# michaelnny/muzero

Measured on AMD Instinct MI355X. Metric: self-play MCTS sims/sec (env-steps/sec = value / sims_per_move), higher is better.
Workload: dtype f32

## Files before the change

### muzero_amd/csrc/mz_env.h

```cpp
#pragma once
#include "mz_device.h"

namespace mz {

constexpr int ENV_CARTPOLE = 1;
constexpr int ENV_TICTACTOE = 2;
constexpr int ENV_GOMOKU = 3;
constexpr int ENV_SYNTHETIC = 4;

struct EnvState {
    int kind, B, A, D, ring_len;
    int bn, nn, win;
    double* cp_state;
    int* steps;
    unsigned int* episode;
    double* init_state;
    signed char* board;
    signed char* planes;
    int* player;
    float* r_obs;
    int* r_action;
    float* r_reward;
    double* r_pi;
    double* r_root;
// ... 471 lines not shown
        if (cell) {
            mine[i] = nm0; mine[nn + i] = m0; mine[2 * nn + i] = m1; mine[3 * nn + i] = m2;
            o[0 * nn + i] = (float)t0; o[1 * nn + i] = (float)nm0;
            o[2 * nn + i] = (float)t1; o[3 * nn + i] = (float)m0;
            o[4 * nn + i] = (float)t2; o[5 * nn + i] = (float)m1;
            o[6 * nn + i] = (float)t3; o[7 * nn + i] = (float)m2;
            o[8 * nn + i] = opp == 1 ? 1.0f : 0.0f;
            if (i == a) { b[i] = (signed char)me; L.mask[(size_t)e * (nn + 1) + a] = 0; }
        }
        if (lane == 0) {
            L.env.player[e] = opp;
            L.env.steps[e] = st + 1;
            L.cur[e] = opp;
            L.opp[e] = me;
        }
    } else {
        if (cell) {
            b[i] = 0;
#pragma unroll
            for (int t = 0; t < 8; t++) { pl[t * nn + i] = 0; o[t * nn + i] = 0.0f; }
            o[8 * nn + i] = 1.0f;
            L.mask[(size_t)e * (nn + 1) + i] = 1;
        }
        if (lane == 0) {
            L.mask[(size_t)e * (nn + 1) + nn] = 1;
            atomicAdd(&L.env.counters[2], 1ULL);
            atomicAdd(&L.env.counters[3], (unsigned long long)(st + 1));
            L.env.steps[e] = 0;
            L.env.episode[e] += 1;
            L.env.player[e] = 1;
            L.cur[e] = 1;
            L.opp[e] = 2;
        }
    }
    const size_t rec = (size_t)L.slot * L.B + e;
    if (lane < A) L.env.r_pi[rec * A + lane] = pi[lane];
    if (lane == 0) {
        L.env.r_action[rec] = a;
        L.env.r_reward[rec] = reward;
        L.env.r_root[rec] = root;
        L.env.r_done[rec] = done ? 1 : 0;
        if (e == 0) {
            atomicAdd(&L.env.counters[0], (unsigned long long)L.B);
            atomicAdd(&L.env.counters[1], (unsigned long long)L.B * (unsigned long long)L.sims);
        }
    }
}

__device__ inline void env_step_group(const EnvLaunch& L, int e, int lane) {
    if (L.env.kind != ENV_TICTACTOE && L.env.kind != ENV_GOMOKU) {
        if (lane == 0) env_step_one(L, e);
        return;
    }
    const int a = __shfl(lane == 0 ? L.action[e] : 0, 0, 16);
    float reward;
    bool done;
    if (L.env.nn <= 16) board_step_small(L, e, lane, a, reward, done);
    else board_step_group(L, e, lane, a, reward, done);
    if (lane == 0) env_record(L, e, a, reward, done);
}

__global__ void k_env_step(const EnvLaunch L) {
    const int g = blockIdx.x * blockDim.x + threadIdx.x;
    if ((g >> 4) < L.B) env_step_group(L, g >> 4, g & 15);
}

struct ReplayRing {
    long long capacity;
    float* state;
    signed char* action;
    int action16;
    float* pi_prob;
    float* value;
    float* reward;
    float* priority;
    long long* num_added;
    long long* ctr;
    int* off;
    int* origin;
    int acc, K, td, board;
    double pw[34];
};

struct EpiLaunch {
    EnvState env;
    ReplayRing ring;
    int B;
    long long move_abs;
};

__device__ inline void epi_emit(const EpiLaunch& E, int e, long long start, int T, int n, long long base, long long keep_from, double* z, int lane) {
    const EnvState& V = E.env;
    const ReplayRing& R = E.ring;
    const int B = E.B, A = V.A, D = V.D, K = R.K;
    auto rec = [&](int i) { return (size_t)((start + i) % V.ring_len) * B + e; };
    if (R.board) {
        const double fr = (double)V.r_reward[rec(T - 1)];
        const int fp = V.r_player[rec(T - 1)];
        for (int t = lane; t < T; t += 64) z[t] = fr != 0.0 ? (V.r_player[rec(t)] == fp ? fr : -fr) : 0.0;
    } else {
        for (int t = lane; t < T; t += 64) {
            double acc = 0.0;
            for (int i = 0; i < R.td; i++) acc = acc + R.pw[i] * (t + i < T ? (double)V.r_reward[rec(t + i)] : 0.0);
            z[t] = acc + R.pw[R.td] * (t + R.td < T ? V.r_root[rec(t + R.td)] : 0.0);
        }
    }
    __syncthreads();
    for (int j = lane; j < n * D; j += 64) {
        const int t = j / D, i = j - t * D;
        if (base + t < keep_from) continue;
        R.state[(size_t)((base + t) % R.capacity) * D + i] = V.r_obs[rec(t) * D + i];
    }
    for (int j = lane; j < n * K; j += 64) {
        const int t = j / K, k = j - t * K, idx = t + k;
        if (base + t < keep_from) continue;
        const size_t o = (size_t)((base + t) % R.capacity) * K + k;
        const bool real = idx < T;
        if (R.action16) reinterpret_cast<short*>(R.action)[o] = real ? (short)V.r_action[rec(idx)] : (short)0;
        else R.action[o] = real ? (signed char)V.r_action[rec(idx)] : (signed char)0;
        R.reward[o] = real ? V.r_reward[rec(idx)] : 0.0f;
        R.value[o] = real ? (float)z[idx] : 0.0f;
    }
    for (int j = lane; j < n * K * A; j += 64) {
        const int t = j / (K * A), r = j - t * K * A, k = r / A, a = r - k * A, idx = t + k;
        if (base + t < keep_from) continue;
        R.pi_prob[((size_t)((base + t) % R.capacity) * K + k) * A + a] = idx < T ? (float)V.r_pi[rec(idx) * A + a] : (float)(1.0 / (double)A);
    }
    for (int t = lane; t < n; t += 64) {
        if (base + t < keep_from) continue;
        const size_t slot = (size_t)((base + t) % R.capacity);
        const double d = V.r_root[rec(t)] - z[t];
        R.priority[slot] = (float)(d < 0.0 ? -d : d);
        if (R.origin) R.origin[slot] = e;
    }
    __syncthreads();
}

__global__ __launch_bounds__(64) void k_epilogue(const EpiLaunch E) {
    extern __shared__ double z[];
    const int e = blockIdx.x, lane = threadIdx.x;
    const EnvState& V = E.env;
    const ReplayRing& R = E.ring;
    long long start = V.ep_start[e];
    int len = (int)(E.move_abs + 1 - start);
    const bool done = V.r_done[(size_t)(E.move_abs % V.ring_len) * E.B + e] != 0;
    const bool flush = !R.board && len == R.acc + R.K + R.td;
    if (flush || done) {
        long long base = R.ctr[0] + (long long)R.off[e];
        const long long keep_from = R.ctr[0] + R.ctr[1] - (long long)R.capacity;
        if (flush) {
            epi_emit(E, e, start, len, R.acc, base, keep_from, z, lane);
            start += R.acc;
            len -= R.acc;
            base += R.acc;
        }
        if (done) {
            epi_emit(E, e, start, len, len, base, keep_from, z, lane);
            start = E.move_abs + 1;
        }
        if (lane == 0) V.ep_start[e] = start;
    }
}

__global__ __launch_bounds__(1024) void k_epi_scan(const EpiLaunch E) {
    __shared__ int part[1024];
    const EnvState& V = E.env;
    const ReplayRing& R = E.ring;
    const int t = threadIdx.x, per = (E.B + 1023) / 1024, e0 = t * per, e1 = e0 + per < E.B ? e0 + per : E.B;
    int sum = 0;
    for (int e = e0; e < e1; e++) {
        int len = (int)(E.move_abs + 1 - V.ep_start[e]);
        const bool done = V.r_done[(size_t)(E.move_abs % V.ring_len) * E.B + e] != 0;
        const bool flush = !R.board && len == R.acc + R.K + R.td;
        int n = 0;
        if (flush) { n += R.acc; len -= R.acc; }
        if (done) n += len;
        R.off[e] = sum;
        sum += n;
    }
    part[t] = sum;
    __syncthreads();
    for (int d = 1; d < 1024; d <<= 1) {
        const int v = t >= d ? part[t - d] : 0;
        __syncthreads();
        part[t] += v;
        __syncthreads();
    }
    const int base = part[t] - sum;
    for (int e = e0; e < e1; e++) R.off[e] += base;
    if (t == 1023) R.ctr[1] = (long long)part[1023];
}

__global__ void k_epi_publish(const ReplayRing R) {
    const long long c = R.ctr[0] + R.ctr[1];
    R.ctr[0] = c;
    *reinterpret_cast<volatile long long*>(R.num_added) = c;
}

}
```

### muzero_amd/csrc/planner.hip

```cpp
#include <hip/hip_runtime.h>

#include <cmath>
#include <cstdio>
#include <cstdlib>
#include <cstring>
#include <map>
#include <string>
#include <vector>

#include "../../include/mzplanner.h"
#include "mz_env.h"
#include "mz_arena.h"
#include "mz_extenv.h"
#include "mz_search.h"
#include "mz_search_fast.h"
#include "mz_convnet.h"

using namespace mz;

static thread_local std::string g_err;

static int fail(int code, const std::string& msg) {
    g_err = msg;
    return code;
// ... 70 lines not shown
    int n_chunks_f32 = 0, n_chunks_w3 = 0;
    PackSrc *d_srcs = nullptr, *h_srcs = nullptr;
    void **d_dst = nullptr, **h_dst = nullptr;
    hipEvent_t ev_in = nullptr, ev_out = nullptr;
    long long bytes_read = 0, bytes_written = 0;
    void free_maps() {
        for (void* b : {(void*)d_map, (void*)d_chunks_f32, (void*)d_chunks_w3, (void*)d_srcs, (void*)d_dst})
            if (b) (void)hipFree(b);
        if (h_srcs) (void)hipHostFree(h_srcs);
        if (h_dst) (void)hipHostFree(h_dst);
        d_map = nullptr; d_chunks_f32 = d_chunks_w3 = nullptr; d_srcs = h_srcs = nullptr; d_dst = h_dst = nullptr;
        n_chunks_f32 = n_chunks_w3 = 0;
        maps_valid = false;
    }
};

struct mz_planner {
    mz_config cfg;
    int device = 0;
    hipStream_t stream = nullptr;
    std::map<std::string, HostTensor> params;
    bool committed = false;

    MlpNet net{};
    MlpLds o{};
    float* d_w[L_COUNT] = {};
    float* d_b[L_COUNT] = {};
    SearchParams sp{};
    SearchParams sp2{};
    bool tree2_ok = false;
    int lds_mode0 = 0, lds_mode2 = 0;
    SearchParams sp2f{};
    bool tree2f_ok = false;
    int lds_mode2f = 0, fast_delta = 0;
    double* d_ftab_tri = nullptr;
    InferParams ip{};
    FastKey fast{};
    bool fast_mse = false;
    bool fast_layout = false;
    bool tree_old = false;
    bool force_generic = false;
    int hwx = -1;
    std::string last_dispatch = "none yet";
    float* d_stream[1] = {};
    float* d_bias_all = nullptr;
    double *d_dbg_noise = nullptr, *d_dbg_utie = nullptr, *d_dbg_ufinal = nullptr;
    FastWeights fw{};

    float* d_obs = nullptr;
    unsigned char* d_mask = nullptr;
    int *d_cur = nullptr, *d_opp = nullptr;
    double* d_temp = nullptr;
    double *d_noise = nullptr, *d_utie = nullptr, *d_ufinal = nullptr;
    float* d_hidden = nullptr;
    double* d_ftab = nullptr;
    int* d_action = nullptr;
    double *d_pi = nullptr, *d_root = nullptr;
    int* d_visits = nullptr;
    int* d_err = nullptr;
    long long* d_stamps = nullptr;
    float *d_spi0 = nullptr, *d_svalues = nullptr, *d_srewards = nullptr;
    int *d_tparent = nullptr, *d_taction = nullptr;
    float *d_inf_in = nullptr, *d_inf_hidden = nullptr, *d_inf_reward = nullptr, *d_inf_value = nullptr, *d_inf_pi = nullptr;
    int* d_inf_action = nullptr;
    int inf_cap = 0;

    bool conv = false;
    bool hbm_tree = false;
    SearchParams spg{};
    float* d_pi_scratch = nullptr;
    ConvNetDev cnet{};
    unsigned char* d_regions = nullptr;
    float *d_pi0 = nullptr, *d_sim_reward = nullptr, *d_sim_value = nullptr;
    const float** d_srcptrs = nullptr;
    float **d_dstptrs = nullptr, **d_rootptrs = nullptr;
    int* d_sim_action = nullptr;

    EnvState env{};
    int env_kind = MZ_ENV_NONE;
    unsigned int move_counter = 0;
    int ring_len = 0, ring_pos = 0, ring_count = 0;
    bool has_replay = false;
    ReplayRing replay{};
    int* d_epi_off = nullptr;
    long long* d_epi_ctr = nullptr;
    long long selfplay_moves = 0;
    ExtEnv ext{};
    int ext_od = 0;
    bool ext_pending = false;
    bool ext_broken = false;
    void* h_ext_frames = nullptr;
    unsigned char *h_ext_mask = nullptr, *h_ext_done = nullptr;
    int *h_ext_cur = nullptr, *h_ext_opp = nullptr, *h_ext_action = nullptr, *h_ext_err = nullptr;
    float* h_ext_reward = nullptr;

    ArenaState arena{};
    bool arena_open = false;
    int arena_ply = 0;
    mz_planner* arena_q = nullptr;
    hipEvent_t ev_arena_pre = nullptr, ev_arena_q = nullptr;

    struct PackState* pk = nullptr;

    bool profiling = false;
    hipEvent_t ev_begin = nullptr, ev_end = nullptr;
    std::vector<std::pair<hipEvent_t, hipEvent_t>> kev;
    size_t kev_used = 0;
};

static int obs_dim(const mz_config& c) { return c.obs_c * c.obs_h * c.obs_w; }
static int pad16(int x) { return (x + 15) & ~15; }

extern "C" const char* mz_last_error(void) { return g_err.c_str(); }
extern "C" const char* mz_version(void) { return "mzplanner 0.1 (gfx950)"; }

static thread_local std::string g_describe;
extern "C" const char* mz_planner_describe(mz_planner* p) {
    if (!p) return "null planner";
    char b[512];
    const ConvSwitches& cs = conv_switches();
    snprintf(b, sizeof b,
             "; switches: MZ_FORCE_GENERIC=%d MZ_HWX=%d MZ_TREE_OLD=%d MZ_HBM_TREE=%d"
             " | per process: MZ_ACTION_SPARSE=%d MZ_ACTION_FUSE=%d MZ_CONV_SPEC=%d MZ_TOWER=%d MZ_CONV_TILE=%d MZ_CONV_G=%d MZ_CONV_NCT=%d",
             (int)p->force_generic, p->hwx, (int)p->tree_old, (int)p->hbm_tree, cs.action_sparse, cs.action_fuse, cs.conv_spec, cs.tower, cs.conv_tile, cs.conv_g, cs.conv_nct);
    g_describe = "search: " + p->last_dispatch + b;
    if (p->conv && p->cnet.split)
        g_describe += std::string(" | conv_precision=bf16x3: ") + split_geometry(p->cnet.hh, p->cnet.hw, p->cnet.P).name + ", one launch per conv";
    else if (p->conv) g_describe += " | conv_precision=f32";
    return g_describe.c_str();
}

static void compute_layout(mz_planner* p) {
    const mz_config& c = p->cfg;
    MlpNet& n = p->net;
    n.in_dim = obs_dim(c); n.A = c.num_actions; n.P = c.num_planes; n.H = c.hidden_dim;
    n.Sv = c.value_support_size; n.Sr = c.reward_support_size;
    n.in_pad = pad16(n.in_dim); n.h_pad = pad16(n.H); n.x_pad = n.h_pad + pad16(n.A); n.p_pad = pad16(n.P);
    const int dims[L_COUNT][2] = {{n.P, n.in_dim}, {n.H, n.P}, {n.P, n.H + n.A}, {n.H, n.P}, {n.P, n.H},
                                  {n.Sr, n.P},     {n.P, n.H}, {n.A, n.P},       {n.P, n.H}, {n.Sv, n.P}};
    for (int l = 0; l < L_COUNT; l++) {
        MlpLayer& L = n.L[l];
        L.n = dims[l][0]; L.k = dims[l][1];
        L.n_tiles = (L.n + 15) / 16;
        if (l == L_DYN0) {
            const int ab = (n.A + 15) / 16, a_last = n.A - 16 * (ab - 1);
            L.kg = n.h_pad / 16 + ab;
            L.last_steps = (a_last + 3) / 4;
        } else {
            L.kg = (L.k + 15) / 16;
            const int rem = L.k - 16 * (L.kg - 1);
            L.last_steps = rem < 4 ? rem : 4;
        }
        L.split = (l == L_REP1 || l == L_DYN1 || l == L_REW1 || l == L_POL1 || l == L_VAL1) ? 1 : 0;
        L.kq = (L.kg + 3) / 4;
    }
    MlpLds& o = p->o;
    int off = 0;
    const int xk = n.in_pad > n.x_pad ? n.in_pad : n.x_pad;
    o.X = off; off += xk * 16;
    o.H1 = off; off += n.p_pad * 16;
    o.V1 = off; off += n.p_pad * 16;
    o.HN = off; off += n.h_pad * 16;
    o.HS = off; off += n.h_pad * 16;
    int mx = n.A; mx = n.Sv > mx ? n.Sv : mx; mx = n.Sr > mx ? n.Sr : mx;
    o.lg_stride = pad16(mx) + 1;
    o.LG = off; off += ((2 * 16 * o.lg_stride + 3) & ~3);
// ... 969 lines not shown
static int upload_roots(mz_planner* p, int batch, const float* h_obs, const uint8_t* h_mask, const int32_t* h_cur, const int32_t* h_opp,
                        const double* h_temp, const mz_rng_inputs* rng, int deterministic) {
    const mz_config& c = p->cfg;
    const size_t B = (size_t)batch, A = (size_t)c.num_actions;
    if (h_obs) HIPCHK(hipMemcpyAsync(p->d_obs, h_obs, B * obs_dim(c) * sizeof(float), hipMemcpyHostToDevice, p->stream));
    if (h_mask) HIPCHK(hipMemcpyAsync(p->d_mask, h_mask, B * A, hipMemcpyHostToDevice, p->stream));
    HIPCHK(hipMemcpyAsync(p->d_cur, h_cur, B * sizeof(int), hipMemcpyHostToDevice, p->stream));
    HIPCHK(hipMemcpyAsync(p->d_opp, h_opp, B * sizeof(int), hipMemcpyHostToDevice, p->stream));
    HIPCHK(hipMemcpyAsync(p->d_temp, h_temp, B * sizeof(double), hipMemcpyHostToDevice, p->stream));
    if (rng) {
        const bool want_noise = !deterministic && c.root_dirichlet_alpha > 0.0 && c.root_exploration_eps > 0.0;
        if (want_noise) {
            if (!rng->h_noise) return fail(MZ_E_INVALID, "rng inputs given but h_noise is NULL while the search mixes Dirichlet noise");
            HIPCHK(hipMemcpyAsync(p->d_noise, rng->h_noise, B * A * sizeof(double), hipMemcpyHostToDevice, p->stream));
        }
        if (!rng->h_u_tie || (!deterministic && !rng->h_u_final)) return fail(MZ_E_INVALID, "rng inputs need h_u_tie and h_u_final");
        HIPCHK(hipMemcpyAsync(p->d_utie, rng->h_u_tie, B * (size_t)c.max_ties * sizeof(double), hipMemcpyHostToDevice, p->stream));
        if (rng->h_u_final) HIPCHK(hipMemcpyAsync(p->d_ufinal, rng->h_u_final, B * sizeof(double), hipMemcpyHostToDevice, p->stream));
    }
    return MZ_OK;
}

static int download_results(mz_planner* p, int batch, int32_t* h_action, double* h_pi, double* h_root, int32_t* h_visits) {
    const size_t B = (size_t)batch, A = (size_t)p->cfg.num_actions;
    int err = 0;
    if (h_action) HIPCHK(hipMemcpyAsync(h_action, p->d_action, B * sizeof(int), hipMemcpyDeviceToHost, p->stream));
    if (h_pi) HIPCHK(hipMemcpyAsync(h_pi, p->d_pi, B * A * sizeof(double), hipMemcpyDeviceToHost, p->stream));
    if (h_root) HIPCHK(hipMemcpyAsync(h_root, p->d_root, B * sizeof(double), hipMemcpyDeviceToHost, p->stream));
    if (h_visits) HIPCHK(hipMemcpyAsync(h_visits, p->d_visits, B * A * sizeof(int), hipMemcpyDeviceToHost, p->stream));
    HIPCHK(hipMemcpyAsync(&err, p->d_err, sizeof(int), hipMemcpyDeviceToHost, p->stream));
    HIPCHK(hipStreamSynchronize(p->stream));
    if (err) {
        HIPCHK(hipMemsetAsync(p->d_err, 0, sizeof(int), p->stream));
        HIPCHK(hipStreamSynchronize(p->stream));
        if (err == 4) return fail(MZ_E_TIES, "injected tie-break stream exhausted (raise mz_config.max_ties)");
        return fail(MZ_E_INVALID, "search kernel reported error " + std::to_string(err));
    }
    return MZ_OK;
}

extern "C" int mz_planner_search(mz_planner* p, int32_t batch, const float* h_obs, const uint8_t* h_mask, const int32_t* h_cur,
                                 const int32_t* h_opp, const double* h_temp, int32_t deterministic, const mz_rng_inputs* rng,
                                 int32_t* h_action, double* h_pi, double* h_root, int32_t* h_visits) {
    if (!p || !h_obs || !h_cur || !h_opp || !h_temp || !h_action || !h_pi || !h_root) return fail(MZ_E_INVALID, "null argument to mz_planner_search");
    if (batch < 1 || batch > p->cfg.num_envs) return fail(MZ_E_INVALID, "batch exceeds mz_config.num_envs");
    if (!p->committed) return fail(MZ_E_STATE, "weights not committed");
    HIPCHK(hipSetDevice(p->device));
    int rc = upload_roots(p, batch, h_obs, h_mask, h_cur, h_opp, h_temp, rng, deterministic);
    if (rc) return rc;
    rc = launch_search(p, batch, deterministic, h_mask != nullptr, rng != nullptr, false);
    if (rc) return rc;
    return download_results(p, batch, h_action, h_pi, h_root, h_visits);
}

extern "C" int mz_planner_search_scripted(mz_planner* p, int32_t batch, const float* h_pi0, const float* h_values, const float* h_rewards,
                                          const uint8_t* h_mask, const int32_t* h_cur, const int32_t* h_opp, const double* h_temp,
                                          int32_t deterministic, const mz_rng_inputs* rng, int32_t* h_action, double* h_pi, double* h_root,
                                          int32_t* h_visits, int32_t* h_tparent, int32_t* h_taction) {
    if (!p || !h_pi0 || !h_values || !h_rewards || !h_cur || !h_opp || !h_temp || !h_action || !h_pi || !h_root)
        return fail(MZ_E_INVALID, "null argument to mz_planner_search_scripted");
    if (batch < 1 || batch > p->cfg.num_envs) return fail(MZ_E_INVALID, "batch exceeds mz_config.num_envs");
    HIPCHK(hipSetDevice(p->device));
    const size_t B = (size_t)p->cfg.num_envs, A = (size_t)p->cfg.num_actions, S = (size_t)p->cfg.num_simulations;
    if (!p->d_spi0) {
        HIPCHK(hipMalloc(&p->d_spi0, B * A * sizeof(float)));
        HIPCHK(hipMalloc(&p->d_svalues, B * S * sizeof(float)));
        HIPCHK(hipMalloc(&p->d_srewards, B * S * sizeof(float)));
        HIPCHK(hipMalloc(&p->d_tparent, B * S * sizeof(int)));
        HIPCHK(hipMalloc(&p->d_taction, B * S * sizeof(int)));
    }
    const size_t b = (size_t)batch;
    HIPCHK(hipMemcpyAsync(p->d_spi0, h_pi0, b * A * sizeof(float), hipMemcpyHostToDevice, p->stream));
    HIPCHK(hipMemcpyAsync(p->d_svalues, h_values, b * S * sizeof(float), hipMemcpyHostToDevice, p->stream));
    HIPCHK(hipMemcpyAsync(p->d_srewards, h_rewards, b * S * sizeof(float), hipMemcpyHostToDevice, p->stream));
    int rc = upload_roots(p, batch, nullptr, h_mask, h_cur, h_opp, h_temp, rng, deterministic);
    if (rc) return rc;
    rc = launch_search(p, batch, deterministic, h_mask != nullptr, rng != nullptr, true);
    if (rc) return rc;
    if (h_tparent) HIPCHK(hipMemcpyAsync(h_tparent, p->d_tparent, b * S * sizeof(int), hipMemcpyDeviceToHost, p->stream));
    if (h_taction) HIPCHK(hipMemcpyAsync(h_taction, p->d_taction, b * S * sizeof(int), hipMemcpyDeviceToHost, p->stream));
    return download_results(p, batch, h_action, h_pi, h_root, h_visits);
}

static void ring_start(mz_planner* p, int max_steps) {
    const mz_config& c = p->cfg;
    p->ring_len = (size_t)c.num_envs * obs_dim(c) * sizeof(float) * 64 > ((size_t)4 << 30) ? 16 : 64;
    if (p->has_replay) {
        const int window = p->replay.acc + p->replay.K + p->replay.td;
        int need = c.is_board_game ? c.num_actions + 1 : window;
        if (max_steps > 0) {
            const int capped = max_steps + (c.is_board_game ? 1 : p->replay.K + p->replay.td);
            need = c.is_board_game ? capped : (window < capped ? window : capped);
        }
        if (need > p->ring_len) p->ring_len = (need + 7) & ~7;
    }
    p->selfplay_moves = 0;
    p->ring_pos = 0;
    p->ring_count = 0;
}

static int ring_finish_move(mz_planner* p) {
    if (p->has_replay) {
        EpiLaunch E{};
        E.env = p->env; E.ring = p->replay; E.B = p->cfg.num_envs; E.move_abs = p->selfplay_moves;
        hipLaunchKernelGGL(k_epi_scan, dim3(1), dim3(1024), 0, p->stream, E);
        hipLaunchKernelGGL(k_epilogue, dim3(p->cfg.num_envs), dim3(64), (size_t)p->ring_len * sizeof(double), p->stream, E);
        hipLaunchKernelGGL(k_epi_publish, dim3(1), dim3(1), 0, p->stream, p->replay);
    }
    HIPCHK(hipGetLastError());
    p->selfplay_moves++;
    p->ring_pos = (p->ring_pos + 1) % p->ring_len;
    if (p->ring_count < p->ring_len) p->ring_count++;
    return MZ_OK;
}

extern "C" int mz_selfplay_reset(mz_planner* p, int32_t env_kind, const double* h_init_state) {
    if (!p) return fail(MZ_E_INVALID, "null planner");
    HIPCHK(hipSetDevice(p->device));
    const mz_config& c = p->cfg;
    int board_n = 3, num_to_win = 3;
    if (env_kind == MZ_ENV_CARTPOLE) {
        if (c.num_actions != 2 || obs_dim(c) != 20) return fail(MZ_E_INVALID, "CartPole env needs num_actions == 2 and a (4,5) observation");
    } else if (env_kind == MZ_ENV_TICTACTOE) {
        if (c.num_actions != 10 || obs_dim(c) != 81) return fail(MZ_E_INVALID, "TicTacToe env needs num_actions == 10 and a (9,3,3) observation");
    } else if (env_kind == MZ_ENV_GOMOKU) {
        if (c.net_kind != MZ_NET_BOARD || c.obs_c != 9 || c.obs_h != c.obs_w || c.num_actions != c.obs_h * c.obs_w + 1 || c.obs_h < 5)
            return fail(MZ_E_INVALID, "Gomoku env needs a board net with a (9,N,N) observation, N >= 5, and num_actions == N*N + 1");
        board_n = c.obs_h;
        num_to_win = 5;
    } else if (env_kind == MZ_ENV_SYNTHETIC) {
        if (h_init_state) return fail(MZ_E_INVALID, "the synthetic env takes no initial state");
    } else {
        return fail(MZ_E_INVALID, "unknown env kind");
    }
    p->env_kind = env_kind;
    p->arena_open = false;
    const int limit = env_kind == MZ_ENV_CARTPOLE ? 500 : (env_kind == MZ_ENV_SYNTHETIC ? 1000 : (1 << 30) - 64);
    ring_start(p, c.is_board_game ? 0 : limit);
    hipError_t e = env_alloc(p->env, env_kind, c.num_envs, c.num_actions, obs_dim(c), p->ring_len, board_n, num_to_win);
    if (e != hipSuccess) return fail(MZ_E_HIP, std::string("env_alloc: ") + hipGetErrorString(e));
    if (h_init_state) HIPCHK(hipMemcpyAsync(p->env.init_state, h_init_state, (size_t)c.num_envs * 4 * sizeof(double), hipMemcpyHostToDevice, p->stream));
    EnvLaunch L{};
    L.env = p->env; L.B = c.num_envs; L.seed = c.seed; L.use_init = h_init_state != nullptr;
    L.obs = p->d_obs; L.mask = p->d_mask; L.cur = p->d_cur; L.opp = p->d_opp;
    hipLaunchKernelGGL(k_env_reset, dim3((c.num_envs + 255) / 256), dim3(256), 0, p->stream, L);
    if (env_kind == MZ_ENV_SYNTHETIC)
        hipLaunchKernelGGL(k_env_synth_obs, dim3(((size_t)c.num_envs * ((obs_dim(c) + 3) / 4) + 255) / 256), dim3(256), 0, p->stream, L);
    HIPCHK(hipGetLastError());
    HIPCHK(hipStreamSynchronize(p->stream));
    return MZ_OK;
}

extern "C" int mz_selfplay_step(mz_planner* p, double temperature, int32_t n_moves) {
    if (!p || n_moves < 1) return fail(MZ_E_INVALID, "bad argument to mz_selfplay_step");
    if (p->arena_open) return fail(MZ_E_STATE, "mz_selfplay_step during an arena: call mz_selfplay_reset first");
    if (p->env_kind == MZ_ENV_NONE) return fail(MZ_E_STATE, "call mz_selfplay_reset first");
    if (p->env_kind == MZ_ENV_EXTERNAL) return fail(MZ_E_STATE, "mz_selfplay_step on host-stepped envs: use mz_selfplay_external_act / _commit");
    if (!p->committed) return fail(MZ_E_STATE, "weights not committed");
    HIPCHK(hipSetDevice(p->device));
    const mz_config& c = p->cfg;
    for (int m = 0; m < n_moves; m++) {
        EnvLaunch L{};
        L.env = p->env; L.B = c.num_envs; L.seed = c.seed; L.temperature = temperature; L.move_counter = p->move_counter;
        L.obs = p->d_obs; L.mask = p->d_mask; L.cur = p->d_cur; L.opp = p->d_opp; L.temp_out = p->d_temp;
        L.action = p->d_action; L.pi = p->d_pi; L.root = p->d_root; L.slot = p->ring_pos; L.sims = c.num_simulations;
        if (!p->conv && !p->hbm_tree && p->env_kind != MZ_ENV_SYNTHETIC) {
            int rc = launch_search(p, c.num_envs, 0, true, false, false, &L);
            if (rc) return rc;
        } else {
            hipLaunchKernelGGL(k_env_pre, dim3((c.num_envs + 255) / 256), dim3(256), 0, p->stream, L);
            HIPCHK(hipMemcpyAsync(p->env.r_obs + (size_t)p->ring_pos * c.num_envs * obs_dim(c), p->d_obs, (size_t)c.num_envs * obs_dim(c) * sizeof(float),
                                  hipMemcpyDeviceToDevice, p->stream));
            int rc = launch_search(p, c.num_envs, 0, true, false, false);
            if (rc) return rc;
            hipLaunchKernelGGL(k_env_step, dim3((c.num_envs + 15) / 16), dim3(256), 0, p->stream, L);
            if (p->env_kind == MZ_ENV_SYNTHETIC)
                hipLaunchKernelGGL(k_env_synth_obs, dim3(((size_t)c.num_envs * ((obs_dim(c) + 3) / 4) + 255) / 256), dim3(256), 0, p->stream, L);
        }
        int rc = ring_finish_move(p);
        if (rc) return rc;
    }
    return MZ_OK;
}

static void ext_free(mz_planner* p) {
    void* dbufs[] = {p->ext.frames, p->ext.hist, p->ext.hist_act, p->ext.head, p->ext.reward, p->ext.done, p->ext.err};
    for (void* b : dbufs)
        if (b) (void)hipFree(b);
    void* hbufs[] = {p->h_ext_frames, p->h_ext_mask, p->h_ext_done, p->h_ext_cur, p->h_ext_opp, p->h_ext_action, p->h_ext_err, p->h_ext_reward};
    for (void* b : hbufs)
        if (b) (void)hipHostFree(b);
    p->ext = ExtEnv{};
    p->h_ext_frames = nullptr; p->h_ext_mask = p->h_ext_done = nullptr;
    p->h_ext_cur = p->h_ext_opp = p->h_ext_action = p->h_ext_err = nullptr;
    p->h_ext_reward = nullptr;
}

static ExtLaunch ext_launch(mz_planner* p, double temperature) {
    const mz_config& c = p->cfg;
    ExtLaunch L{};
    L.env = p->env; L.x = p->ext; L.B = c.num_envs; L.A = c.num_actions; L.OD = p->ext_od;
    L.slot = p->ring_pos; L.prev_slot = (p->ring_pos + p->ring_len - 1) % p->ring_len; L.first = p->selfplay_moves == 0;
    L.parity = (int)(p->selfplay_moves & 1); L.sims = c.num_simulations; L.check = p->has_replay ? 1 : 0; L.move_abs = p->selfplay_moves;
    L.temperature = temperature; L.obs = p->d_obs; L.cur = p->d_cur; L.temp_out = p->d_temp;
    L.action = p->d_action; L.pi = p->d_pi; L.root = p->d_root;
    return L;
}

extern "C" int mz_selfplay_reset_external(mz_planner* p, const mz_external_env* x) {
    if (!p || !x) return fail(MZ_E_INVALID, "null argument to mz_selfplay_reset_external");
    HIPCHK(hipSetDevice(p->device));
    const mz_config& c = p->cfg;
    const int S = x->stack_history;
    if (S < 0 || x->frame_c < 1 || x->frame_h < 1 || x->frame_w < 1 || x->max_episode_steps < 0 || x->temp_switch_steps < 0)
        return fail(MZ_E_INVALID, "mz_external_env: stack_history >= 0, frame dimensions >= 1, max_episode_steps >= 0, temp_switch_steps >= 0");
    if (!x->is_obs_image && (x->frame_h != 1 || x->frame_w != 1))
        return fail(MZ_E_INVALID, "mz_external_env: vector frames are frame_c = D, frame_h = frame_w = 1");
    const long long FE = (long long)x->frame_c * x->frame_h * x->frame_w;
    const long long stacked = S == 0 ? FE : (x->is_obs_image ? (long long)S * (x->frame_c + 1) * x->frame_h * x->frame_w : (long long)S * (x->frame_c + 1));
    if (stacked != obs_dim(c))
        return fail(MZ_E_INVALID, "mz_external_env: the stacked observation has " + std::to_string(stacked) + " values, the network's (obs_c*obs_h*obs_w) " +
                                      std::to_string(obs_dim(c)));
    if (S == 0 && x->frame_u8) return fail(MZ_E_INVALID, "mz_external_env: frame_u8 needs stack_history > 0 (whole observations are float32)");
    ext_free(p);
    p->arena_open = false;
    p->env_kind = MZ_ENV_EXTERNAL;
    p->ext_pending = p->ext_broken = false;
    ring_start(p, x->max_episode_steps);
    hipError_t e = env_alloc(p->env, ENV_EXTERNAL, c.num_envs, c.num_actions, obs_dim(c), p->ring_len, 3, 3);
    if (e != hipSuccess) return fail(MZ_E_HIP, std::string("env_alloc: ") + hipGetErrorString(e));
    ExtEnv& X = p->ext;
    X.S = S; X.image = x->is_obs_image ? 1 : 0; X.C = x->frame_c; X.HW = x->frame_h * x->frame_w; X.FE = (int)FE; X.u8 = x->frame_u8 ? 1 : 0;
    X.temp_steps = x->temp_switch_steps > 0 ? x->temp_switch_steps : (c.num_actions <= 10 ? 6 : 30);
    p->ext_od = obs_dim(c);
    const size_t B = (size_t)c.num_envs, fbytes = (size_t)FE * (X.u8 ? 1 : 4);
    HIPCHK(hipMalloc(&X.frames, B * fbytes));
    if (S > 0) {
        HIPCHK(hipMalloc(&X.hist, B * S * fbytes));
        HIPCHK(hipMalloc(&X.hist_act, B * S * sizeof(int)));
        HIPCHK(hipMalloc(&X.head, 2 * B * sizeof(int)));
        HIPCHK(hipMemsetAsync(X.head, 0, 2 * B * sizeof(int), p->stream));
    }
    HIPCHK(hipMalloc(&X.reward, B * sizeof(float)));
    HIPCHK(hipMalloc(&X.done, B));
    HIPCHK(hipMalloc(&X.err, sizeof(int)));
    HIPCHK(hipHostMalloc(&p->h_ext_frames, B * fbytes, hipHostMallocDefault));
    HIPCHK(hipHostMalloc(reinterpret_cast<void**>(&p->h_ext_mask), B * c.num_actions, hipHostMallocDefault));
    HIPCHK(hipHostMalloc(reinterpret_cast<void**>(&p->h_ext_cur), B * sizeof(int), hipHostMallocDefault));
    HIPCHK(hipHostMalloc(reinterpret_cast<void**>(&p->h_ext_opp), B * sizeof(int), hipHostMallocDefault));
    HIPCHK(hipHostMalloc(reinterpret_cast<void**>(&p->h_ext_action), B * sizeof(int), hipHostMallocDefault));
    HIPCHK(hipHostMalloc(reinterpret_cast<void**>(&p->h_ext_reward), B * sizeof(float), hipHostMallocDefault));
// ... 32 lines not shown
    HIPCHK(hipGetLastError());
    int rc = launch_search(p, c.num_envs, 0, true, false, false);
    if (rc) return rc;
    hipLaunchKernelGGL(k_ext_record, dim3((c.num_envs * c.num_actions + 255) / 256), dim3(256), 0, p->stream, L);
    HIPCHK(hipGetLastError());
    int err = 0;
    HIPCHK(hipMemcpyAsync(p->h_ext_action, p->d_action, B * sizeof(int), hipMemcpyDeviceToHost, p->stream));
    HIPCHK(hipMemcpyAsync(&err, p->d_err, sizeof(int), hipMemcpyDeviceToHost, p->stream));
    HIPCHK(hipStreamSynchronize(p->stream));
    if (err) {
        HIPCHK(hipMemsetAsync(p->d_err, 0, sizeof(int), p->stream));
        HIPCHK(hipStreamSynchronize(p->stream));
        return fail(MZ_E_INVALID, "search kernel reported error " + std::to_string(err));
    }
    std::memcpy(h_action, p->h_ext_action, B * sizeof(int));
    p->ext_pending = true;
    return MZ_OK;
}

extern "C" int mz_selfplay_external_commit(mz_planner* p, const float* h_reward, const uint8_t* h_done) {
    if (!p || !h_reward || !h_done) return fail(MZ_E_INVALID, "null argument to mz_selfplay_external_commit");
    if (p->env_kind != MZ_ENV_EXTERNAL) return fail(MZ_E_STATE, "call mz_selfplay_reset_external first");
    if (p->ext_broken) return fail(MZ_E_STATE, "a commit found an over-long trajectory: call mz_selfplay_reset_external");
    if (!p->ext_pending) return fail(MZ_E_STATE, "mz_selfplay_external_commit without an mz_selfplay_external_act");
    HIPCHK(hipSetDevice(p->device));
    const mz_config& c = p->cfg;
    const size_t B = (size_t)c.num_envs;
    std::memcpy(p->h_ext_reward, h_reward, B * sizeof(float));
    std::memcpy(p->h_ext_done, h_done, B);
    HIPCHK(hipMemcpyAsync(p->ext.reward, p->h_ext_reward, B * sizeof(float), hipMemcpyHostToDevice, p->stream));
    HIPCHK(hipMemcpyAsync(p->ext.done, p->h_ext_done, B, hipMemcpyHostToDevice, p->stream));
    const ExtLaunch L = ext_launch(p, 0.0);
    hipLaunchKernelGGL(k_ext_commit, dim3((c.num_envs + 255) / 256), dim3(256), 0, p->stream, L);
    HIPCHK(hipGetLastError());
    p->ext_pending = false;
    if (p->has_replay) {
        HIPCHK(hipMemcpyAsync(p->h_ext_err, p->ext.err, sizeof(int), hipMemcpyDeviceToHost, p->stream));
        HIPCHK(hipStreamSynchronize(p->stream));
        if (*p->h_ext_err != INT_MAX) {
            p->ext_broken = true;
            return fail(MZ_E_INVALID, "env " + std::to_string(*p->h_ext_err) + ": open trajectory of more than " + std::to_string(p->ring_len) +
                                          " moves outgrew the record ring (raise mz_external_env.max_episode_steps); no items written, reset next");
        }
    }
    return ring_finish_move(p);
}

extern "C" int mz_selfplay_attach_replay(mz_planner* p, const mz_replay_ring* ring) {
    if (!p) return fail(MZ_E_INVALID, "null planner");
    HIPCHK(hipSetDevice(p->device));
    HIPCHK(hipStreamSynchronize(p->stream));
    if (!ring) {
        p->has_replay = false;
        return MZ_OK;
    }
    const mz_config& c = p->cfg;
    if (ring->capacity < 1 || !ring->state || !ring->action || !ring->pi_prob || !ring->value || !ring->reward || !ring->priority || !ring->num_added)
        return fail(MZ_E_INVALID, "mz_replay_ring: capacity and every array but `origin` are required");
    if (ring->unroll_steps < 1 || ring->td_steps < 0 || ring->td_steps > 32 || ring->acc_seq_length < 1)
        return fail(MZ_E_INVALID, "mz_replay_ring: unroll_steps >= 1, 0 <= td_steps <= 32, acc_seq_length >= 1");
    {
        const void* ptrs[8] = {ring->state, ring->action, ring->pi_prob, ring->value, ring->reward, ring->priority, ring->num_added, ring->origin};
        static const char* names[8] = {"state", "action", "pi_prob", "value", "reward", "priority", "num_added", "origin"};
        for (int i = 0; i < 8; i++) {
            if (!ptrs[i]) continue;
            hipPointerAttribute_t at{};
            const hipError_t e = hipPointerGetAttributes(&at, ptrs[i]);
            if (e != hipSuccess || at.type != hipMemoryTypeDevice || at.device != p->device) {
                (void)hipGetLastError();
                return fail(MZ_E_INVALID, std::string("mz_replay_ring.") + names[i] + " is not memory of the planner's GPU");
            }
        }
    }
    ReplayRing& R = p->replay;
    R.capacity = ring->capacity; R.state = ring->state; R.action = reinterpret_cast<signed char*>(ring->action); R.action16 = c.num_actions > 128 ? 1 : 0; R.pi_prob = ring->pi_prob;
    R.value = ring->value; R.reward = ring->reward; R.priority = ring->priority; R.num_added = reinterpret_cast<long long*>(ring->num_added);
    R.origin = ring->origin; R.acc = ring->acc_seq_length; R.K = ring->unroll_steps; R.td = ring->td_steps; R.board = c.is_board_game;
    for (int i = 0; i <= R.td; i++) R.pw[i] = std::pow(c.discount, (double)i);
    if (!p->d_epi_ctr) HIPCHK(hipMalloc(&p->d_epi_ctr, 2 * sizeof(long long)));
    HIPCHK(hipMemsetAsync(p->d_epi_ctr, 0, 2 * sizeof(long long), p->stream));
    HIPCHK(hipMemcpyAsync(p->d_epi_ctr, R.num_added, sizeof(long long), hipMemcpyDeviceToDevice, p->stream));
    HIPCHK(hipStreamSynchronize(p->stream));
    R.ctr = p->d_epi_ctr;
    if (!p->d_epi_off) HIPCHK(hipMalloc(&p->d_epi_off, (size_t)c.num_envs * sizeof(int)));
    R.off = p->d_epi_off;
    p->has_replay = true;
    p->arena_open = false;
    p->env_kind = MZ_ENV_NONE;
    return MZ_OK;
}

extern "C" int mz_selfplay_read(mz_planner* p, int32_t n_moves, float* h_obs, int32_t* h_action, float* h_reward, double* h_pi,
                                double* h_root, int32_t* h_player, uint8_t* h_done) {
    if (!p || n_moves < 1 || n_moves > p->ring_count) return fail(MZ_E_INVALID, "n_moves exceeds the recorded history");
    HIPCHK(hipSetDevice(p->device));
    HIPCHK(hipStreamSynchronize(p->stream));
    const size_t B = (size_t)p->cfg.num_envs, A = (size_t)p->cfg.num_actions, D = (size_t)obs_dim(p->cfg);
    const int first = ((p->ring_pos - n_moves) % p->ring_len + p->ring_len) % p->ring_len;
    const int n1 = n_moves < p->ring_len - first ? n_moves : p->ring_len - first;
    for (int part = 0; part < 2; part++) {
        const size_t slot = part == 0 ? (size_t)first : 0, cnt = part == 0 ? (size_t)n1 : (size_t)(n_moves - n1), done_moves = part == 0 ? 0 : (size_t)n1;
        if (cnt == 0) continue;
        if (h_obs) HIPCHK(hipMemcpyAsync(h_obs + done_moves * B * D, p->env.r_obs + slot * B * D, cnt * B * D * sizeof(float), hipMemcpyDeviceToHost, p->stream));
        if (h_action) HIPCHK(hipMemcpyAsync(h_action + done_moves * B, p->env.r_action + slot * B, cnt * B * sizeof(int), hipMemcpyDeviceToHost, p->stream));
        if (h_reward) HIPCHK(hipMemcpyAsync(h_reward + done_moves * B, p->env.r_reward + slot * B, cnt * B * sizeof(float), hipMemcpyDeviceToHost, p->stream));
        if (h_pi) HIPCHK(hipMemcpyAsync(h_pi + done_moves * B * A, p->env.r_pi + slot * B * A, cnt * B * A * sizeof(double), hipMemcpyDeviceToHost, p->stream));
        if (h_root) HIPCHK(hipMemcpyAsync(h_root + done_moves * B, p->env.r_root + slot * B, cnt * B * sizeof(double), hipMemcpyDeviceToHost, p->stream));
        if (h_player) HIPCHK(hipMemcpyAsync(h_player + done_moves * B, p->env.r_player + slot * B, cnt * B * sizeof(int), hipMemcpyDeviceToHost, p->stream));
        if (h_done) HIPCHK(hipMemcpyAsync(h_done + done_moves * B, p->env.r_done + slot * B, cnt * B, hipMemcpyDeviceToHost, p->stream));
    }
    HIPCHK(hipStreamSynchronize(p->stream));
    return MZ_OK;
}

extern "C" int mz_selfplay_counters(mz_planner* p, int64_t out[4]) {
    if (!p || !out) return fail(MZ_E_INVALID, "null argument");
    if (p->env_kind == MZ_ENV_NONE || p->arena_open) return fail(MZ_E_STATE, "call mz_selfplay_reset first");
    HIPCHK(hipSetDevice(p->device));
    HIPCHK(hipStreamSynchronize(p->stream));
    unsigned long long c[4];
    HIPCHK(hipMemcpy(c, p->env.counters, sizeof(c), hipMemcpyDeviceToHost));
    for (int i = 0; i < 4; i++) out[i] = (int64_t)c[i];
    return MZ_OK;
}

static bool arena_same_config(const mz_config& a, const mz_config& b) {
    mz_config x = a, y = b;
    x.seed = y.seed = 0;
    return x.net_kind == y.net_kind && x.obs_c == y.obs_c && x.obs_h == y.obs_h && x.obs_w == y.obs_w && x.num_actions == y.num_actions &&
           x.num_planes == y.num_planes && x.hidden_dim == y.hidden_dim && x.num_res_blocks == y.num_res_blocks &&
           x.value_support_size == y.value_support_size && x.reward_support_size == y.reward_support_size &&
           x.num_simulations == y.num_simulations && x.discount == y.discount && x.pb_c_base == y.pb_c_base && x.pb_c_init == y.pb_c_init &&
           x.is_board_game == y.is_board_game && x.has_known_bounds == y.has_known_bounds && x.known_bounds_min == y.known_bounds_min &&
           x.known_bounds_max == y.known_bounds_max && x.root_dirichlet_alpha == y.root_dirichlet_alpha &&
           x.root_exploration_eps == y.root_exploration_eps && x.num_envs == y.num_envs && x.max_ties == y.max_ties &&
           x.legacy_scalar_promotion == y.legacy_scalar_promotion && x.conv_precision == y.conv_precision;
}

static ArenaLaunch arena_launch(mz_planner* p) {
    const mz_config& c = p->cfg;
    ArenaLaunch R{};
    R.L.env = p->env; R.L.B = c.num_envs; R.L.seed = c.seed; R.L.sims = c.num_simulations;
    R.L.obs = p->arena.obs; R.L.mask = p->arena.mask; R.L.cur = p->arena.cur; R.L.opp = p->arena.opp;
    R.a = p->arena;
    R.ply = p->arena_ply;
    return R;
}

static void arena_seg_searched(ArenaSeg& g, mz_planner* s) {
    g.obs = s->d_obs; g.mask = s->d_mask; g.cur = s->d_cur; g.opp = s->d_opp; g.temp = s->d_temp;
    g.action = s->d_action; g.pi = s->d_pi; g.root = s->d_root;
}

extern "C" int mz_arena_reset(mz_planner* p, int32_t env_kind, int32_t opponent_kind, mz_planner* q, int32_t opening_plies, const double* h_init_state) {
    if (!p) return fail(MZ_E_INVALID, "null planner");
    const mz_config& c = p->cfg;
    int board_n = 3, num_to_win = 3;
    if (env_kind == MZ_ENV_CARTPOLE) {
        if (c.num_actions != 2 || obs_dim(c) != 20) return fail(MZ_E_INVALID, "CartPole env needs num_actions == 2 and a (4,5) observation");
    } else if (env_kind == MZ_ENV_TICTACTOE) {
        if (c.num_actions != 10 || obs_dim(c) != 81) return fail(MZ_E_INVALID, "TicTacToe env needs num_actions == 10 and a (9,3,3) observation");
    } else if (env_kind == MZ_ENV_GOMOKU) {
        if (c.net_kind != MZ_NET_BOARD || c.obs_c != 9 || c.obs_h != c.obs_w || c.num_actions != c.obs_h * c.obs_w + 1 || c.obs_h < 5)
            return fail(MZ_E_INVALID, "Gomoku env needs a board net with a (9,N,N) observation, N >= 5, and num_actions == N*N + 1");
        board_n = c.obs_h;
        num_to_win = 5;
    } else {
// ... 287 lines not shown
```

Before: 294.1 million.

## Batch replay epilogue over chunks of moves to cut per-move kernel launches

Instead of launching the scan, epilogue and publish kernels after every self-play move, moves are accumulated and processed every N moves (default 8, set by MZ_EPI_CHUNK) by new chunked kernels. These walk episode boundaries across several moves using a done bitmask and a prefix scan over a larger offset buffer. The ring length is enlarged so older slots stay valid until the chunk is flushed. This trades three launches per move for three per chunk, at the cost of more ring memory and delayed replay publication.

Result: no change. 294.2 million, median of 2 (+0.0%).

```diff
diff --git a/muzero_amd/csrc/mz_env.h b/muzero_amd/csrc/mz_env.h
--- a/muzero_amd/csrc/mz_env.h
+++ b/muzero_amd/csrc/mz_env.h
@@ -577,6 +577,8 @@
     double pw[34];
 };
 
+constexpr int EPI_CHUNK_MAX = 64;
+
 struct EpiLaunch {
     EnvState env;
     ReplayRing ring;
@@ -686,6 +688,89 @@
     if (t == 1023) R.ctr[1] = (long long)part[1023];
 }
 
+
+__device__ inline void epi_walk(const ReplayRing& R, long long move, bool done, long long& start, int& n_flush, int& n_done) {
+    int len = (int)(move + 1 - start);
+    const bool flush = !R.board && len == R.acc + R.K + R.td;
+    n_flush = n_done = 0;
+    if (flush) { n_flush = R.acc; len -= R.acc; start += R.acc; }
+    if (done) { n_done = len; start = move + 1; }
+}
+
+__device__ inline int epi_slot(const EpiLaunch& E, int slot0, int j) { return slot0 + j < E.env.ring_len ? slot0 + j : slot0 + j - E.env.ring_len; }
+
+__global__ __launch_bounds__(1024) void k_epi_scan_chunk(const EpiLaunch E, const int n) {
+    __shared__ int part[1024];
+    const ReplayRing& R = E.ring;
+    const int t = threadIdx.x, slot0 = (int)(E.move_abs % E.env.ring_len);
+    for (int e = t; e < E.B; e += 1024) {
+        unsigned long long dm = 0;
+#pragma unroll 8
+        for (int j = 0; j < n; j++) dm |= (unsigned long long)(E.env.r_done[(size_t)epi_slot(E, slot0, j) * E.B + e] != 0) << j;
+        long long start = E.env.ep_start[e];
+        for (int j = 0; j < n; j++) {
+            int nf, nd;
+            epi_walk(R, E.move_abs + j, (dm >> j) & 1, start, nf, nd);
+            R.off[(size_t)j * E.B + e] = nf + nd;
+        }
+    }
+    __syncthreads();
+    const int N = n * E.B, per = (N + 1023) / 1024, i0 = t * per < N ? t * per : N, i1 = i0 + per < N ? i0 + per : N;
+    int sum = 0;
+#pragma unroll 8
+    for (int i = i0; i < i1; i++) sum += R.off[i];
+    part[t] = sum;
+    __syncthreads();
+    for (int d = 1; d < 1024; d <<= 1) {
+        const int v = t >= d ? part[t - d] : 0;
+        __syncthreads();
+        part[t] += v;
+        __syncthreads();
+    }
+    int run = part[t] - sum;
+    int i = i0;
+    for (; i + 8 <= i1; i += 8) {
+        int c[8];
+#pragma unroll
+        for (int k = 0; k < 8; k++) c[k] = R.off[i + k];
+#pragma unroll
+        for (int k = 0; k < 8; k++) { R.off[i + k] = run; run += c[k]; }
+    }
+    for (; i < i1; i++) {
+        const int c = R.off[i];
+        R.off[i] = run;
+        run += c;
+    }
+    if (t == 1023) R.ctr[1] = (long long)part[1023];
+}
+
+__global__ __launch_bounds__(64) void k_epilogue_chunk(const EpiLaunch E, const int n) {
+    extern __shared__ double z[];
+    const int e = blockIdx.x, lane = threadIdx.x;
+    const ReplayRing& R = E.ring;
+    const int slot0 = (int)(E.move_abs % E.env.ring_len);
+    const unsigned long long dm = __ballot(lane < n && E.env.r_done[(size_t)epi_slot(E, slot0, lane < n ? lane : 0) * E.B + e] != 0);
+    const long long start0 = E.env.ep_start[e];
+    long long start = start0, ctr0 = 0, keep_from = 0;
+    bool first = true;
+    for (int j = 0; j < n; j++) {
+        const long long move = E.move_abs + j, s = start;
+        int nf, nd;
+        epi_walk(R, move, (dm >> j) & 1, start, nf, nd);
+        if (nf + nd == 0) continue;
+        if (first) {
+            ctr0 = R.ctr[0];
+            keep_from = ctr0 + R.ctr[1] - (long long)R.capacity;
+            first = false;
+        }
+        const long long base = ctr0 + (long long)R.off[(size_t)j * E.B + e];
+        const int len = (int)(move + 1 - s);
+        if (nf) epi_emit(E, e, s, len, nf, base, keep_from, z, lane);
+        if (nd) epi_emit(E, e, s + nf, nd, nd, base + nf, keep_from, z, lane);
+    }
+    if (lane == 0 && start != start0) E.env.ep_start[e] = start;
+}
+
 __global__ void k_epi_publish(const ReplayRing R) {
     const long long c = R.ctr[0] + R.ctr[1];
     R.ctr[0] = c;
diff --git a/muzero_amd/csrc/planner.hip b/muzero_amd/csrc/planner.hip
--- a/muzero_amd/csrc/planner.hip
+++ b/muzero_amd/csrc/planner.hip
@@ -176,6 +176,7 @@
     int ring_len = 0, ring_pos = 0, ring_count = 0;
     bool has_replay = false;
     ReplayRing replay{};
+    int epi_chunk = 1;
     int* d_epi_off = nullptr;
     long long* d_epi_ctr = nullptr;
     long long selfplay_moves = 0;
@@ -1311,9 +1312,10 @@
     return download_results(p, batch, h_action, h_pi, h_root, h_visits);
 }
 
-static void ring_start(mz_planner* p, int max_steps) {
+static void ring_start(mz_planner* p, int max_steps, int chunk = 1) {
     const mz_config& c = p->cfg;
     p->ring_len = (size_t)c.num_envs * obs_dim(c) * sizeof(float) * 64 > ((size_t)4 << 30) ? 16 : 64;
+    p->epi_chunk = 1;
     if (p->has_replay) {
         const int window = p->replay.acc + p->replay.K + p->replay.td;
         int need = c.is_board_game ? c.num_actions + 1 : window;
@@ -1321,11 +1323,22 @@
             const int capped = max_steps + (c.is_board_game ? 1 : p->replay.K + p->replay.td);
             need = c.is_board_game ? capped : (window < capped ? window : capped);
         }
-        if (need > p->ring_len) p->ring_len = (need + 7) & ~7;
+        const int plain = need > p->ring_len ? (need + 7) & ~7 : p->ring_len;
+        const size_t slot_bytes = (size_t)c.num_envs * ((size_t)obs_dim(c) * sizeof(float) + (size_t)c.num_actions * sizeof(double) + 21);
+        auto len_for = [&](int ch) { return need + ch - 1 > plain ? (need + ch - 1 + 7) & ~7 : plain; };
+        while (chunk > 1 && (size_t)(len_for(chunk) - plain) * slot_bytes > ((size_t)64 << 20)) chunk--;
+        p->epi_chunk = chunk < 1 ? 1 : chunk;
+        p->ring_len = len_for(p->epi_chunk);
     }
     p->selfplay_moves = 0;
     p->ring_pos = 0;
     p->ring_count = 0;
+}
+
+static void ring_advance(mz_planner* p) {
+    p->selfplay_moves++;
+    p->ring_pos = (p->ring_pos + 1) % p->ring_len;
+    if (p->ring_count < p->ring_len) p->ring_count++;
 }
 
 static int ring_finish_move(mz_planner* p) {
@@ -1337,9 +1350,17 @@
         hipLaunchKernelGGL(k_epi_publish, dim3(1), dim3(1), 0, p->stream, p->replay);
     }
     HIPCHK(hipGetLastError());
-    p->selfplay_moves++;
-    p->ring_pos = (p->ring_pos + 1) % p->ring_len;
-    if (p->ring_count < p->ring_len) p->ring_count++;
+    ring_advance(p);
+    return MZ_OK;
+}
+
+static int ring_finish_chunk(mz_planner* p, int n) {
+    EpiLaunch E{};
+    E.env = p->env; E.ring = p->replay; E.B = p->cfg.num_envs; E.move_abs = p->selfplay_moves - n;
+    hipLaunchKernelGGL(k_epi_scan_chunk, dim3(1), dim3(1024), 0, p->stream, E, n);
+    hipLaunchKernelGGL(k_epilogue_chunk, dim3(p->cfg.num_envs), dim3(64), (size_t)p->ring_len * sizeof(double), p->stream, E, n);
+    hipLaunchKernelGGL(k_epi_publish, dim3(1), dim3(1), 0, p->stream, p->replay);
+    HIPCHK(hipGetLastError());
     return MZ_OK;
 }
 
@@ -1365,7 +1386,13 @@
     p->env_kind = env_kind;
     p->arena_open = false;
     const int limit = env_kind == MZ_ENV_CARTPOLE ? 500 : (env_kind == MZ_ENV_SYNTHETIC ? 1000 : (1 << 30) - 64);
-    ring_start(p, c.is_board_game ? 0 : limit);
+    int chunk = 1;
+    if (p->has_replay && !p->conv && !p->hbm_tree && env_kind != MZ_ENV_SYNTHETIC) {
+        const char* ec = getenv("MZ_EPI_CHUNK");
+        chunk = ec ? atoi(ec) : 8;
+        chunk = chunk < 1 ? 1 : (chunk > EPI_CHUNK_MAX ? EPI_CHUNK_MAX : chunk);
+    }
+    ring_start(p, c.is_board_game ? 0 : limit, chunk);
     hipError_t e = env_alloc(p->env, env_kind, c.num_envs, c.num_actions, obs_dim(c), p->ring_len, board_n, num_to_win);
     if (e != hipSuccess) return fail(MZ_E_HIP, std::string("env_alloc: ") + hipGetErrorString(e));
     if (h_init_state) HIPCHK(hipMemcpyAsync(p->env.init_state, h_init_state, (size_t)c.num_envs * 4 * sizeof(double), hipMemcpyHostToDevice, p->stream));
@@ -1388,6 +1415,8 @@
     if (!p->committed) return fail(MZ_E_STATE, "weights not committed");
     HIPCHK(hipSetDevice(p->device));
     const mz_config& c = p->cfg;
+    const bool chunked = p->has_replay && p->epi_chunk > 1;
+    int pending = 0;
     for (int m = 0; m < n_moves; m++) {
         EnvLaunch L{};
         L.env = p->env; L.B = c.num_envs; L.seed = c.seed; L.temperature = temperature; L.move_counter = p->move_counter;
@@ -1395,7 +1424,20 @@
         L.action = p->d_action; L.pi = p->d_pi; L.root = p->d_root; L.slot = p->ring_pos; L.sims = c.num_simulations;
         if (!p->conv && !p->hbm_tree && p->env_kind != MZ_ENV_SYNTHETIC) {
             int rc = launch_search(p, c.num_envs, 0, true, false, false, &L);
-            if (rc) return rc;
+            if (rc) {
+                if (pending) (void)ring_finish_chunk(p, pending);
+                return rc;
+            }
+            if (chunked) {
+                HIPCHK(hipGetLastError());
+                ring_advance(p);
+                if (++pending == p->epi_chunk || m + 1 == n_moves) {
+                    rc = ring_finish_chunk(p, pending);
+                    if (rc) return rc;
+                    pending = 0;
+                }
+                continue;
+            }
         } else {
             hipLaunchKernelGGL(k_env_pre, dim3((c.num_envs + 255) / 256), dim3(256), 0, p->stream, L);
             HIPCHK(hipMemcpyAsync(p->env.r_obs + (size_t)p->ring_pos * c.num_envs * obs_dim(c), p->d_obs, (size_t)c.num_envs * obs_dim(c) * sizeof(float),
@@ -1594,7 +1636,7 @@
     HIPCHK(hipMemcpyAsync(p->d_epi_ctr, R.num_added, sizeof(long long), hipMemcpyDeviceToDevice, p->stream));
     HIPCHK(hipStreamSynchronize(p->stream));
     R.ctr = p->d_epi_ctr;
-    if (!p->d_epi_off) HIPCHK(hipMalloc(&p->d_epi_off, (size_t)c.num_envs * sizeof(int)));
+    if (!p->d_epi_off) HIPCHK(hipMalloc(&p->d_epi_off, (size_t)(p->conv || p->hbm_tree ? 1 : EPI_CHUNK_MAX) * c.num_envs * sizeof(int)));
     R.off = p->d_epi_off;
     p->has_replay = true;
     p->arena_open = false;
```
